# ay-lab/fithic

Measured on AMD Instinct MI355X. Metric: contact-pairs/sec through spline+p-value+BH pass (5 kb cis, whole node), higher is better.
Workload: dtype f64

## Files before the change

### fithic_amd/_capi.py

```python
import ctypes
import os
import subprocess

import numpy as np

from . import _loader

_PKG = os.path.dirname(os.path.abspath(__file__))
LIB_PATH = _loader.LIB_PATH
CSRC = os.path.join(_PKG, "csrc")

FHX_OK = 0
FHX_ERR_ARG, FHX_ERR_NO_DEVICE, FHX_ERR_HIP, FHX_ERR_UNSUPPORTED, FHX_ERR_REFERENCE_EXIT, FHX_ERR_NOMEM, FHX_ERR_INTERNAL = -1, -2, -3, -4, -5, -6, -7
MODE_INTRA_ONLY, MODE_INTER_ONLY, MODE_ALL = 0, 1, 2
TOTALS_REFERENCE, TOTALS_WIDE = 0, 1
INT64_MAX = (1 << 63) - 1

(A_HIST_SUMCC, A_HIST_NPAIRS, A_BIN_LB, A_BIN_UB, A_BIN_POSS, A_BIN_SUMCC, A_BIN_SUMDIST, A_BIN_POSS7, A_X, A_Y,
 A_KNOTS, A_COEFFS, A_TABLE_X, A_TABLE_Y0, A_TABLE_Y, A_OUTLIER_DIST_HIST, A_FDR_COUNTS, A_BIN_POSS0, A_DIST_KEYS,
 A_OUTLIER_DISTS) = range(20)
_ARRAY_DTYPE = {A_BIN_SUMDIST: np.float64, A_X: np.float64, A_Y: np.float64, A_KNOTS: np.float64,
                A_COEFFS: np.float64, A_TABLE_Y0: np.float64, A_TABLE_Y: np.float64}


# ... 73 lines not shown
    "fhx_reset_passes": (ctypes.c_int, [_P]),
    "fhx_get_stats": (ctypes.c_int, [_P, ctypes.POINTER(FhxStats)]),
    "fhx_fetch": (ctypes.c_int, [_P, _F64P, _F64P, _F64P, _F64P, _F64P]),
    "fhx_fetch_flags": (ctypes.c_int, [_P, ctypes.POINTER(ctypes.c_uint8), ctypes.POINTER(ctypes.c_uint8)]),
    "fhx_fetch_outlier_rows": (ctypes.c_int, [_P, ctypes.POINTER(ctypes.c_int64), ctypes.c_int64, ctypes.POINTER(ctypes.c_int64)]),
    "fhx_get_array": (ctypes.c_int, [_P, ctypes.c_int, _P, ctypes.c_int64, _I64P]),
    "fhx_device_ptr": (_P, [_P, ctypes.c_int]),
    "fhx_n_sorted": (ctypes.c_int64, [_P]),
    "fhx_bh_sort_stats": (ctypes.c_int, [_P, _I64P]),
    "fhx_k3_pass_info": (ctypes.c_int, [_P, _I64P]),
    "fhx_debug_k3_tiles_per_group": (ctypes.c_int, [_P, ctypes.c_int]),
    "fhx_debug_k1_wide": (ctypes.c_int, [_P, ctypes.c_int]),
    "fhx_k3_compact_variant": (ctypes.c_int, [_P, ctypes.POINTER(ctypes.c_int32)]),
    "fhx_kernel_seconds": (ctypes.c_int, [_P, _F64P, _F64P, _F64P]),
    "fhx_kernel_seconds_total": (ctypes.c_int, [_P, _F64P, _I64P, ctypes.c_int]),
    "fhx_kernel_events_dropped": (ctypes.c_int, [_P, _I64P]),
    "fhx_k2_heavy_launch": (ctypes.c_int, [_P, _F64P, _I64P]),
    "fhx_k2_heavy_clock": (ctypes.c_int, [_P, _F64P]),
    "fhx_k2_class_rows": (ctypes.c_int, [_P, _I64P]),
    "fhx_bdtrc_array": (ctypes.c_int, [_P, ctypes.c_double, _I32P, _F64P, ctypes.c_int64, _F64P]),
    "fhx_debug_format": (ctypes.c_int, [_P, _F64P, ctypes.c_int64, ctypes.c_int32, ctypes.c_char_p, _I32P]),
    "fhx_debug_contfrac": (ctypes.c_int, [_P, ctypes.c_int, ctypes.c_int, _F64P, _F64P, _F64P, ctypes.c_int64, _F64P]),
    "fhx_debug_lean_div": (ctypes.c_int, [_P, _F64P, _F64P, ctypes.c_int64, _F64P]),
    "fhx_debug_classify": (ctypes.c_int, [_P, ctypes.c_double, _I32P, _F64P, ctypes.c_int64, _I32P, _I32P, _F64P]),
    "fhx_debug_k2_rows": (ctypes.c_int, [_P, ctypes.c_double, ctypes.c_double, _I32P, _F64P, ctypes.POINTER(ctypes.c_uint8), ctypes.c_int64,
                                         ctypes.c_int32, _F64P, _I64P, _I64P, _I64P, ctypes.c_int64]),
    "fhx_bh_array": (ctypes.c_int, [_P, _F64P, ctypes.c_int64, ctypes.c_double, _F64P]),
    "fhx_bh_top_hist": (ctypes.c_int, [_P, _I64P, ctypes.c_int64]),
    "fhx_bh_set_cutoff": (ctypes.c_int, [_P, _I64P, ctypes.c_int64, ctypes.c_double]),
    "fhx_bh_top_hist_device": (ctypes.c_int, [_P]),
    "fhx_bh_set_cutoff_device": (ctypes.c_int, [_P, ctypes.c_double]),
    "fhx_bh_local_sort": (ctypes.c_int, [_P]),
    "fhx_bh_apply_sorted": (ctypes.c_int, [_P, _P, ctypes.c_int64, ctypes.c_int64, ctypes.c_double, ctypes.c_double, _P, _F64P]),
    "fhx_sort_u64": (ctypes.c_int, [_P, _P, ctypes.c_int64, _P, _P]),
    "fhx_bh_scatter": (ctypes.c_int, [_P, _P]),
    "fhx_memcpy_d2d": (ctypes.c_int, [_P, _P, _P, ctypes.c_int64]),
    "fhx_comm_unique_id": (ctypes.c_int, [_P, ctypes.c_int64]),
    "fhx_comm_init": (ctypes.c_int, [_P, _P, ctypes.c_int, ctypes.c_int]),
    "fhx_comm_init_custom": (ctypes.c_int, [_P, _P, ctypes.c_int, ctypes.c_int]),
    "fhx_comm_destroy": (ctypes.c_int, [_P]),
    "fhx_comm_info": (ctypes.c_int, [_P, ctypes.POINTER(ctypes.c_int), ctypes.POINTER(ctypes.c_int), ctypes.POINTER(ctypes.c_int)]),
    "fhx_run_pass_distributed": (ctypes.c_int, [_P, ctypes.POINTER(FhxFitInfo)]),
    "fhx_next_pass_distributed": (ctypes.c_int, [_P, _I64P]),
    "fhx_pass_stats_distributed": (ctypes.c_int, [_P, ctypes.POINTER(FhxStats)]),
    "fhx_bh_distributed": (ctypes.c_int, [_P, ctypes.c_double]),
    "fhx_dist_stage_seconds": (ctypes.c_int, [_P, _F64P]),
# ... 696 lines not shown
        return p, by_class, redo.value, hist

    def debug_contfrac(self, kind, lazy, a, b, x):
        a, b, x = (np.ascontiguousarray(v, np.float64) for v in (a, b, x))
        out = np.empty(len(a), np.float64)
        self._check(self._L.fhx_debug_contfrac(self._h, int(kind), int(lazy), _ptr(a, ctypes.c_double), _ptr(b, ctypes.c_double),
                                               _ptr(x, ctypes.c_double), len(a), _ptr(out, ctypes.c_double)))
        return out

    def debug_format(self, values, kind):
        v = np.ascontiguousarray(values, np.float64)
        text = ctypes.create_string_buffer(len(v) * 32)
        ln = np.empty(len(v), np.int32)
        self._check(self._L.fhx_debug_format(self._h, _ptr(v, ctypes.c_double), len(v), int(kind), text, _ptr(ln, ctypes.c_int32)))
        raw = text.raw
        return [raw[32 * i:32 * i + ln[i]] if ln[i] > 0 else None for i in range(len(v))]

    def debug_lean_div(self, n, d):
        n, d = (np.ascontiguousarray(v, np.float64) for v in (n, d))
        out = np.empty(len(n), np.float64)
        self._check(self._L.fhx_debug_lean_div(self._h, _ptr(n, ctypes.c_double), _ptr(d, ctypes.c_double), len(n), _ptr(out, ctypes.c_double)))
        return out

    def bh_array(self, p, n_total_tests):
        p = np.ascontiguousarray(p, np.float64)
        q = np.empty(len(p), np.float64)
        self._check(self._L.fhx_bh_array(self._h, _ptr(p, ctypes.c_double), len(p), float(n_total_tests), _ptr(q, ctypes.c_double)))
        return q

    def bh_top_hist(self):
        h = np.zeros(8192, np.int64)
        self._check(self._L.fhx_bh_top_hist(self._h, _ptr(h, ctypes.c_int64), len(h)))
        return h

    def bh_set_cutoff(self, global_hist, n_total_tests):
        h = np.ascontiguousarray(global_hist, np.int64)
        self._check(self._L.fhx_bh_set_cutoff(self._h, _ptr(h, ctypes.c_int64), len(h), float(n_total_tests)))

    def bh_top_hist_device(self):
        self._check(self._L.fhx_bh_top_hist_device(self._h))
        return self.device_ptr(4)

    def bh_set_cutoff_device(self, n_total_tests):
        self._check(self._L.fhx_bh_set_cutoff_device(self._h, float(n_total_tests)))

    def bh_local_sort(self):
# ... 668 lines not shown
```

### fithic_amd/csrc/fhx_bdtrc.hpp

```cpp
#pragma once
#include <hip/hip_runtime.h>
#include <cstdint>

namespace fhx {
namespace dev {

constexpr double kMachEp = 1.11022302462515654042E-16;
constexpr double kMaxLog = 7.09782712893383996732E2;
constexpr double kMinLog = -7.451332191019412076235E2;
constexpr double kMaxGam = 171.624376956302725;
constexpr double kBig = 4.503599627370496e15;
constexpr double kBigInv = 2.22044604925031308085e-16;

struct BinomTables {
    const double* lbeta;
    const double* inv_beta;
    double n;
    int small_n;
};

__device__ __forceinline__ double cephes_log1p(double x) {
    double z = 1.0 + x;
    if (z < 0.70710678118654752440 || z > 1.41421356237309504880) return log(z);
    z = x * x;
// ... 13 lines not shown
    z = -0.5 * z + x * (z * num / den);
    return x + z;
}

__device__ __forceinline__ double cephes_expm1(double x) {
    if (!isfinite(x)) {
        if (isnan(x) || x > 0) return x;
        return -1.0;
    }
    if (x < -0.5 || x > 0.5) return exp(x) - 1.0;
    const double xx = x * x;
    double ep = 1.2617719307481059087798E-4;
    ep = ep * xx + 3.0299440770744196129956E-2;
    ep = ep * xx + 9.9999999999999999991025E-1;
    double r = x * ep;
    double eq = 3.0019850513866445504159E-6;
    eq = eq * xx + 2.5244834034968410419224E-3;
    eq = eq * xx + 2.2726554820815502876593E-1;
    eq = eq * xx + 2.0000000000000000000897E0;
    r = r / (eq - r);
    return r + r;
}

template <bool SMALL_N = true>
__device__ __forceinline__ double pseries(double a, double b, double x, double lbeta_ab, double inv_beta_ab) {
    const double ai = 1.0 / a;
    double u = (1.0 - b) * x;
    double v = u / (a + 1.0);
    const double t1 = v;
    double t = u;
    double n = 2.0;
    double s = 0.0;
    const double z = kMachEp * ai;
    while (fabs(v) > z) {
        u = (n - b) * x / n;
        t *= u;
        v = t / (a + n);
        s += v;
        n += 1.0;
    }
    s += t1;
    s += ai;
    u = a * log(x);
    if (SMALL_N && (a + b) < kMaxGam && fabs(u) < kMaxLog) {
        t = inv_beta_ab;
        s = s * t * pow(x, a);
    } else {
        t = -lbeta_ab + u + log(s);
        s = (t < kMinLog) ? 0.0 : exp(t);
    }
    return s;
}

template <int KIND>
__device__ __forceinline__ double contfrac(double a, double b, double x) {
    double k1, k2, k3, k4, k5, k6, k7, k8, arg;
    if (KIND == 0) {
        arg = x;
        k1 = a; k2 = a + b; k3 = a; k4 = a + 1.0; k5 = 1.0; k6 = b - 1.0; k7 = k4; k8 = a + 2.0;
    } else {
        arg = x / (1.0 - x);
        k1 = a; k2 = b - 1.0; k3 = a; k4 = a + 1.0; k5 = 1.0; k6 = a + b; k7 = a + 1.0; k8 = a + 2.0;
    }
// ... 20 lines not shown
            t = 1.0;
        }
        if (t < thresh) break;

        k1 += 1.0;
        k2 += (KIND == 0) ? 1.0 : -1.0;
        k3 += 2.0;
        k4 += 2.0;
        k5 += 1.0;
        k6 += (KIND == 0) ? -1.0 : 1.0;
        k7 += 2.0;
        k8 += 2.0;

        if ((fabs(qk) + fabs(pk)) > kBig) {
            pkm2 *= kBigInv; pkm1 *= kBigInv; qkm2 *= kBigInv; qkm1 *= kBigInv;
        }
        if ((fabs(qk) < kBigInv) || (fabs(pk) < kBigInv)) {
            pkm2 *= kBig; pkm1 *= kBig; qkm2 *= kBig; qkm1 *= kBig;
        }
    } while (++n < 300);
    return ans;
}

__device__ __forceinline__ double lean_div(double n, double d) {
    const double y0 = __builtin_amdgcn_rcp(d);
    const double e0 = __builtin_fma(-d, y0, 1.0);
    const double y1 = __builtin_fma(y0, e0, y0);
    const double e1 = __builtin_fma(-d, y1, 1.0);
    const double y2 = __builtin_fma(y1, e1, y1);
    const double q0 = n * y2;
    const double r0 = __builtin_fma(-d, q0, n);
    return __builtin_fma(r0, y2, q0);
}

template <int MODE>
__device__ __forceinline__ double cf_div(double n, double d, double& y) {
    if (MODE == 0) return n / d;
    if (MODE == 1) return lean_div(n, d);
    double e = __builtin_fma(-d, y, 1.0);
    y = __builtin_fma(y, e, y);
    if (MODE == 2) {
        e = __builtin_fma(-d, y, 1.0);
        y = __builtin_fma(y, e, y);
    }
    const double q0 = n * y;
    const double r0 = __builtin_fma(-d, q0, n);
    return __builtin_fma(r0, y, q0);
}

template <int KIND, int MODE>
__device__ __forceinline__ double contfrac_lazy_impl(double a, double b, double arg) {
    double k1, k2, k3, k4, k5, k6, k8;
    if (KIND == 0) {
        k1 = a; k2 = a + b; k3 = a; k4 = a + 1.0; k5 = 1.0; k6 = b - 1.0; k8 = a + 2.0;
    } else {
        k1 = a; k2 = b - 1.0; k3 = a; k4 = a + 1.0; k5 = 1.0; k6 = a + b; k8 = a + 2.0;
    }
    double pkm2 = 0.0, qkm2 = 1.0, pkm1 = 1.0, qkm1 = 1.0;
    double rp = 1.0, rq = 1.0;
    double ans = 1.0, r = 1.0;
    bool fast_ok = true;
    const double thresh = 3.0 * kMachEp;
    double yrec = 0.0;
    if (MODE >= 2) {
        const double d0 = k3 * k4;
        yrec = __builtin_amdgcn_rcp(d0);
        double e0 = __builtin_fma(-d0, yrec, 1.0);
        yrec = __builtin_fma(yrec, e0, yrec);
        if (MODE == 3) {
            e0 = __builtin_fma(-d0, yrec, 1.0);
            yrec = __builtin_fma(yrec, e0, yrec);
        }
    }
    int n = 0;
    do {
        double xk = -cf_div<MODE>(arg * k1 * k2, k3 * k4, yrec);
        double pk = pkm1 + pkm2 * xk;
        double qk = qkm1 + qkm2 * xk;
        pkm2 = pkm1; pkm1 = pk; qkm2 = qkm1; qkm1 = qk;

        xk = cf_div<MODE>(arg * k5 * k6, k4 * k8, yrec);
        pk = pkm1 + pkm2 * xk;
        qk = qkm1 + qkm2 * xk;
        pkm2 = pkm1; pkm1 = pk; qkm2 = qkm1; qkm1 = qk;

        const double apk = fabs(pk), aqk = fabs(qk);
        const double mag_sum = aqk + apk;
        const double mag_min = fmin(apk, aqk);
        bool exact = true;
        if (__builtin_expect(fast_ok && mag_min > 1e-100 && mag_sum < 1e100, 1)) {
            const double c1 = rp * qk;
            const double c2 = pk * rq;
            if (__builtin_expect(fabs(c1 - c2) > 1e-13 * fabs(c2), 1)) {
                rp = pk;
                rq = qk;
                exact = false;
            }
        }
        if (__builtin_expect(exact, 0)) {
            if (fast_ok) {
                ans = rp / rq;
                r = ans;
            }
            double t;
            if (qk != 0) r = pk / qk;
            if (r != 0) {
                t = fabs((ans - r) / r);
                ans = r;
            } else {
                t = 1.0;
            }
            if (ans != r) fast_ok = false;
            rp = ans;
            rq = 1.0;
            if (t < thresh) break;
        }

        k1 += 1.0;
        k2 += (KIND == 0) ? 1.0 : -1.0;
        k3 += 2.0;
        k4 += 2.0;
        k5 += 1.0;
        k6 += (KIND == 0) ? -1.0 : 1.0;
        k8 += 2.0;

        if (__builtin_expect(mag_sum > kBig, 0)) {
            pkm2 *= kBigInv; pkm1 *= kBigInv; qkm2 *= kBigInv; qkm1 *= kBigInv;
        }
        if (__builtin_expect(mag_min < kBigInv, 0)) {
            pkm2 *= kBig; pkm1 *= kBig; qkm2 *= kBig; qkm1 *= kBig;
        }
    } while (++n < 300);
    return fast_ok ? rp / rq : ans;
}

template <int KIND>
__device__ __forceinline__ double contfrac_lazy(double a, double b, double x) {
    const double arg = (KIND == 0) ? x : x / (1.0 - x);
    const double aa = fabs(arg);
    if (aa > 1e-150 && aa < 1e150 && a >= 1.0 && a < 4.5e15 && b < 4.5e15) {
        if (a >= 2e8) return contfrac_lazy_impl<KIND, 3>(a, b, arg);
        if (a >= 1e6) return contfrac_lazy_impl<KIND, 2>(a, b, arg);
        return contfrac_lazy_impl<KIND, 1>(a, b, arg);
    }
    return contfrac_lazy_impl<KIND, 0>(a, b, arg);
}

struct CfRow {
    double k1, k2, k5, k6, d0, y0, d1, y1;
};
constexpr int kCfIters = 300;
constexpr double kCfLazyT = 1e-15;

typedef const CfRow __attribute__((address_space(4))) * CfRowConstPtr;

typedef double cf_d8 __attribute__((ext_vector_type(8)));
__device__ __forceinline__ CfRow cf_load_row(CfRowConstPtr p0) {
    const volatile cf_d8 __attribute__((address_space(4))) * p = (const volatile cf_d8 __attribute__((address_space(4))) *)p0;
    const cf_d8 v = *p;
    CfRow r;
    r.k1 = v[0]; r.k2 = v[1]; r.k5 = v[2]; r.k6 = v[3];
    r.d0 = v[4]; r.y0 = v[5]; r.d1 = v[6]; r.y1 = v[7];
    __builtin_amdgcn_sched_barrier(0);
    return r;
}

// ... 431 lines not shown
                                                double lbeta_ab, double inv_beta_ab) {
    double y = a * log(x);
    double t = b * log(xc);
    if (SMALL_N && (a + b) < kMaxGam && fabs(y) < kMaxLog && fabs(t) < kMaxLog) {
        t = pow(xc, b);
        t *= pow(x, a);
        t /= a;
        t *= w;
        t *= inv_beta_ab;
    } else {
        y += t - lbeta_ab;
        y += log(w / a);
        t = (y < kMinLog) ? 0.0 : exp(y);
    }
    if (flag == 1) {
        if (t <= kMachEp)
            t = 1.0 - kMachEp;
        else
            t = 1.0 - t;
    }
    return t;
}

template <int CLS, bool SMALL_N = true>
__device__ __forceinline__ double bdtrc_count_class(int count, const BinomTables& T, double p) {
    const double fk = (double)count - 1.0;
    const double aa = fk + 1.0, bb = T.n - fk, xx = p;
    const double lb = T.lbeta[count];
    const double ib = (SMALL_N && T.small_n) ? T.inv_beta[count] : 0.0;
    if (CLS == BC_PSERIES) {
        if (bb * xx <= 1.0 && xx <= 0.95) return pseries<SMALL_N>(aa, bb, xx, lb, ib);
        const double w = 1.0 - xx;
        double t = pseries<SMALL_N>(bb, aa, w, lb, ib);
        return (t <= kMachEp) ? 1.0 - kMachEp : 1.0 - t;
    }
    const double w1 = 1.0 - xx;
    if (CLS == BC_CF_BCF) return incbet_finish<SMALL_N>(aa, bb, xx, w1, contfrac_lazy<0>(aa, bb, xx), 0, lb, ib);
    if (CLS == BC_CF_SWAPPED) return incbet_finish<SMALL_N>(bb, aa, w1, xx, contfrac_lazy<0>(bb, aa, w1), 1, lb, ib);
    const int flag = (xx > aa / (aa + bb)) ? 1 : 0;
    const double a = flag ? bb : aa, b = flag ? aa : bb, x = flag ? w1 : xx, xc = flag ? xx : w1;
    return incbet_finish<SMALL_N>(a, b, x, xc, contfrac_lazy<1>(a, b, x) / xc, flag, lb, ib);
}

}
}
```

### fithic_amd/csrc/fhx_k2.hip

```cpp
#include "fhx_ctx.hpp"

namespace fhx {

__device__ __forceinline__ double prior_by_search(const K2Params& P, long long dist) {
    double look = (double)dist;
    if (look < P.min_x) look = P.min_x;
    if (look > P.max_x) look = P.max_x;
    int lo = 0, hi = P.n_table;
    while (lo < hi) {
        const int mid = (lo + hi) >> 1;
        if (P.table_x[mid] < look)
            lo = mid + 1;
        else
            hi = mid;
    }
    return P.table_y[min(lo, P.n_table - 1)];
}

template <int NF = -1>
__device__ __forceinline__ bool row_prior(const K2Params& P, int l1, int l2, double& prior, bool& is_inter) {
    const bool inter = l2 < 0;
    const int s2 = inter ? ~l2 : l2;
    const double b1 = P.no_bias ? 1.0 : P.slot_bias[l1], b2 = P.no_bias ? 1.0 : P.slot_bias[s2];
    if ((b1 < 0 || b2 < 0) && !inter) return false;
// ... 363 lines not shown
    }
    __device__ __forceinline__ Cursor open(unsigned int v) const {
        Cursor c;
        c.pr = pair_of(v);
        load(c);
        return c;
    }
    __device__ __forceinline__ const QEntry* at(const QSpan& q, Cursor& c, unsigned int v) const {
        if (v >= c.end) {
            do ++c.pr;
            while (v >= prefix[c.pr + 1]);
            load(c);
        }
        const unsigned int u = v - c.base;
        return u < c.c0 ? qentry(q, 2 * c.pr, (long long)u) : qentry(q, 2 * c.pr + 1, (long long)(u - c.c0));
    }
};
constexpr int K2_WAVES = K2_THREADS / 64;

template <int CLS, bool SMALL_N>
__global__ __launch_bounds__(K2_THREADS) void k2_queue(K2Params P, QSpan q) {
    __shared__ unsigned int hist_lds[K2_HIST_BINS];
    __shared__ unsigned int prefix_lds[QDense::PAIRS + 1], wave_tot[K2_WAVES];
    FusedHist H;
    H.init(hist_lds, P.top_hist);
    QDense D;
    D.build(q, prefix_lds, wave_tot);
    const unsigned long long total = D.total();
    const unsigned int lane = threadIdx.x & 63;
    const unsigned long long n_waves = (unsigned long long)gridDim.x * K2_WAVES;
    const unsigned long long share = ((total + n_waves - 1) / n_waves + 63ull) & ~63ull;
    const unsigned long long begin = ((unsigned long long)blockIdx.x * K2_WAVES + (threadIdx.x >> 6)) * share;
    const unsigned long long end = min(total, begin + share);
    QDense::Cursor cur{0, 0u, 0u, 0u};
    if (begin + lane < end) cur = D.open((unsigned int)(begin + lane));
#pragma unroll 1
    for (unsigned long long v = begin + lane; v < end; v += 64) {
        const QEntry e = *D.at(q, cur, (unsigned int)v);
        const bool is_inter = e.count < 0;
        const int c = is_inter ? -e.count : e.count;
        const double pv = dev::bdtrc_count_class<CLS, SMALL_N>(c, is_inter ? P.inter : P.intra, e.prior);
        store_p<false>(P.p + e.row, pv);
        H.add(pv);
    }
    H.flush(P.top_hist);
}

constexpr int K2_SORT_TILE = 1024;
constexpr int K2_SORT_BUCKETS = 32;
template <int CLS, bool SMALL_N, int WPE>
__global__ __launch_bounds__(K2_THREADS) __attribute__((amdgpu_waves_per_eu(WPE))) void k2_queue_by_count(K2Params P, QSpan q,
                                                                                                         unsigned int* next_tile) {
    static_assert(K2_SORT_TILE == 4 * K2_THREADS, "four entries per thread");
    __shared__ QEntry tile[K2_SORT_TILE];
    __shared__ unsigned int bucket_cnt[K2_SORT_BUCKETS], bucket_off[K2_SORT_BUCKETS];
    __shared__ unsigned int hist_lds[K2_HIST_BINS];
    __shared__ unsigned int prefix_lds[QDense::PAIRS + 1], wave_tot[K2_WAVES], tile_lds;
    FusedHist H;
    H.init(hist_lds, P.top_hist);
    QDense D;
    D.build(q, prefix_lds, wave_tot);
    const unsigned int total = D.total();
    const unsigned int share = (total + gridDim.x - 1) / gridDim.x;
    const unsigned int rounds = max(1u, (share + K2_SORT_TILE - 1) / K2_SORT_TILE);
    const unsigned int tile_n = max(min((unsigned int)K2_SORT_TILE, ((share + rounds - 1) / rounds + 63u) & ~63u), 64u);
    const unsigned int tiles = (total + tile_n - 1) / tile_n;
    unsigned int mine = blockIdx.x;
    for (;;) {
        if (threadIdx.x < K2_SORT_BUCKETS) bucket_cnt[threadIdx.x] = 0;
        if (threadIdx.x == 0) tile_lds = mine;
        __syncthreads();
        const unsigned int t = tile_lds;
        if (t >= tiles) break;
        if (threadIdx.x == 0) mine = gridDim.x + atomicAdd(next_tile, 1u);
        const unsigned int v0 = t * tile_n;
        const int m = (int)min(tile_n, total - v0);
        QEntry e[4];
        int bucket[4];
        unsigned int slot[4];
        QDense::Cursor cur{0, 0u, 0u, 0u};
// ... 7 lines not shown
                const int c = e[r].count < 0 ? -e[r].count : e[r].count;
                bucket[r] = c < K2_SORT_BUCKETS - 1 ? c : K2_SORT_BUCKETS - 1;
                slot[r] = atomicAdd(&bucket_cnt[bucket[r]], 1u);
            }
        }
        __syncthreads();
        if (threadIdx.x < K2_SORT_BUCKETS) {
            unsigned int off = 0;
            for (int b = 0; b < (int)threadIdx.x; ++b) off += bucket_cnt[b];
            bucket_off[threadIdx.x] = off;
        }
        __syncthreads();
#pragma unroll
        for (int r = 0; r < 4; ++r)
            if (bucket[r] >= 0) tile[bucket_off[bucket[r]] + slot[r]] = e[r];
        __syncthreads();
#pragma unroll 1
        for (int r = 0; r < 4; ++r) {
            const int idx = r * K2_THREADS + threadIdx.x;
            if (idx < m) {
                const QEntry x = tile[idx];
                const bool is_inter = x.count < 0;
                const int c = is_inter ? -x.count : x.count;
                const double pv = dev::bdtrc_count_class<CLS, SMALL_N>(c, is_inter ? P.inter : P.intra, x.prior);
                store_p<false>(P.p + x.row, pv);
                H.add(pv);
            }
        }
        __syncthreads();
    }
    H.flush(P.top_hist);
}



__device__ __forceinline__ int k2h_bucket(int signed_count) {
    const bool inter = signed_count < 0;
    const int c = inter ? -signed_count : signed_count;
    return c < K2H_KCAP ? (inter ? K2H_KCAP + c : c) : K2H_GENERIC;
}

__global__ __launch_bounds__(K2H_THREADS) void k2h_scatter(QSpan q, const unsigned int* __restrict__ block_hist,
                                                           const unsigned int* __restrict__ off, QEntry* __restrict__ out) {
    __shared__ unsigned int cursor[K2H_BUCKETS];
    for (int d = threadIdx.x; d < K2H_BUCKETS; d += K2H_THREADS) cursor[d] = off[d] + block_hist[(size_t)d * K2H_BLOCKS + blockIdx.x];
    __syncthreads();
    for (int sh = blockIdx.x; sh < q.n_shards; sh += K2H_BLOCKS) {
// ... 180 lines not shown
    unsigned long long at = tile_offsets[blockIdx.x] + fhxscan::block_exclusive_scan(c, &total);
    for (int k = 0; k < fhxscan::SCAN_ITEMS; ++k)
        if (base + k < n && flag[base + k]) rows[at++] = base + k;
}

__global__ void k_bdtrc_array(dev::BinomTables T, const int32_t* __restrict__ count, const double* __restrict__ prior,
                              int64_t n, double* __restrict__ out) {
    const int64_t stride = (int64_t)gridDim.x * blockDim.x;
    for (int64_t i = (int64_t)blockIdx.x * blockDim.x + threadIdx.x; i < n; i += stride)
        out[i] = dev::bdtrc_count(count[i], T, prior[i]);
}

template <int KIND, int LAZY>
__global__ void k_debug_contfrac(const double* __restrict__ a, const double* __restrict__ b, const double* __restrict__ x,
                                 int64_t n, double* __restrict__ out) {
    const int64_t stride = (int64_t)gridDim.x * blockDim.x;
    for (int64_t i = (int64_t)blockIdx.x * blockDim.x + threadIdx.x; i < n; i += stride)
        out[i] = LAZY ? dev::contfrac_lazy<KIND>(a[i], b[i], x[i]) : dev::contfrac<KIND>(a[i], b[i], x[i]);
}

__global__ void k_debug_lean_div(const double* __restrict__ n, const double* __restrict__ d, int64_t len, double* __restrict__ out) {
    const int64_t stride = (int64_t)gridDim.x * blockDim.x;
    for (int64_t i = (int64_t)blockIdx.x * blockDim.x + threadIdx.x; i < len; i += stride) out[i] = dev::lean_div(n[i], d[i]);
}

__global__ __launch_bounds__(256) void k2_memo_rows(int n_d, int lo_idx, int cap, int with_inter, int32_t* __restrict__ loc1,
                                                   int32_t* __restrict__ loc2, int32_t* __restrict__ count, int64_t n_v) {
    const int64_t stride = (int64_t)gridDim.x * blockDim.x;
    const int64_t intra = (int64_t)n_d * (cap + 1);
    for (int64_t i = (int64_t)blockIdx.x * blockDim.x + threadIdx.x; i < n_v; i += stride) {
        if (i < intra) {
            const int d = lo_idx + (int)(i / (cap + 1));
            loc1[i] = 0;
            loc2[i] = d;
            count[i] = (int)(i % (cap + 1));
        } else {
            loc1[i] = 0;
            loc2[i] = ~0;
            count[i] = (int)(i - intra);
        }
        (void)with_inter;
    }
}

__global__ __launch_bounds__(256) void k2_memo_gather(K2Params P, const double* __restrict__ table, int n_d, int cap, int has_intra,
                                                     int has_inter, unsigned int* __restrict__ overflow_rows,
// ... 227 lines not shown
    static_assert((K2H_BLOCKS & (K2H_BLOCKS - 1)) == 0, "shard -> column by masking");
    Q->heavy_hist = plan.legacy_heavy ? nullptr : ctx->d_block_hist;
    if (Q->heavy_hist && !prezeroed)
        FHX_HIP(hipMemsetAsync(ctx->d_block_hist, 0, (size_t)K2H_BUCKETS * K2H_BLOCKS * sizeof(unsigned int), ctx->stream));
    ctx->k2_shards = plan.n_shards;
    auto span = [&](int cls, QEntry* buf, int dir) {
        Q->q[cls - 1] = QSpan{dir > 0 ? buf : buf + plan.cap_s - 1, plan.cap_s, dir, plan.n_shards, Q->count + (size_t)(cls - 1) * K2_MAX_SHARDS};
    };
    span(dev::BC_CF_SWAPPED, ctx->d_queue[0], 1);
    span(dev::BC_PSERIES, ctx->d_queue[0], -1);
    span(dev::BC_CF_BCF, ctx->d_queue[1], 1);
    span(dev::BC_CF_BD, ctx->d_queue[1], -1);
    span(K2_CLOSED, ctx->d_queue_sorted, 1);
    return FHX_OK;
}

template <int CLS, bool SMALL_N>
static void launch_k2_queue(fhx_ctx* ctx, const K2Params& P, const K2Queues& Q) {
    hipLaunchKernelGGL(HIP_KERNEL_NAME(k2_queue<CLS, SMALL_N>), dim3(2 * resident_grid(ctx, k2_queue<CLS, SMALL_N>)), dim3(K2_THREADS), 0,
                       ctx->stream, P, Q.q[CLS - 1]);
}
template <int CLS, bool SMALL_N>
static void launch_k2_queue_by_count(fhx_ctx* ctx, const K2Params& P, const K2Queues& Q) {
    constexpr int PIECE = SMALL_N ? 4 : 5;
    hipLaunchKernelGGL(HIP_KERNEL_NAME(k2_queue_by_count<CLS, SMALL_N, PIECE>), dim3(resident_grid(ctx, k2_queue_by_count<CLS, SMALL_N, PIECE>)),
                       dim3(K2_THREADS), 0, ctx->stream, P, Q.q[CLS - 1], (unsigned int*)(ctx->d_words->k2_next + CLS));
}
template <int ROWS, int WAVES, bool SMALL_N>
static void launch_k2h_heavy(fhx_ctx* ctx, const K2Params& P, QEntry* redo) {
    hipLaunchKernelGGL(HIP_KERNEL_NAME(k2h_heavy<ROWS, WAVES, SMALL_N>), dim3(256 * WAVES), dim3(K2H_THREADS), 0, ctx->stream,
                       K2HeavyParams{P.intra, P.inter, P.p, P.top_hist}, (const QEntry*)ctx->d_queue_sorted, (const unsigned int*)ctx->d_k2h_off,
                       (const unsigned int*)ctx->d_digit_total, (const dev::CfRow*)ctx->d_cf_tab, redo, &ctx->d_words->k2_redo,
                       (unsigned int*)ctx->d_words->k2_next);
}

template <bool SMALL_N>
static int launch_k2(fhx_ctx* ctx, const K2Plan& plan, const K2Params& P, const K2Queues& Q) {
    const dim3 cgrid(plan.n_shards), block(K2_THREADS);
    if (P.nonfixed)
        hipLaunchKernelGGL(HIP_KERNEL_NAME(k2_classify<1, 4, 0>), cgrid, block, 0, ctx->stream, P, Q);
    else
        hipLaunchKernelGGL(HIP_KERNEL_NAME(k2_classify<0, 4, 3, true, true>), cgrid, block, 0, ctx->stream, P, Q);
    hipLaunchKernelGGL(k2_closed, dim3(256 * 8), block, 0, ctx->stream, P, Q.q[K2_CLOSED - 1], &ctx->d_words->k2_redo, &ctx->d_words->bh_cutoff);
    if (plan.legacy_heavy) {
        FHX_HIP(hipEventRecord(ctx->ev[6], ctx->stream));
        launch_k2_queue<dev::BC_CF_SWAPPED, SMALL_N>(ctx, P, Q);
        FHX_HIP(hipEventRecord(ctx->ev[7], ctx->stream));
// ... 298 lines not shown
    if (thr5) FHX_HIP(hipMemcpyAsync(thr5, d_thr, (size_t)n * 40, hipMemcpyDeviceToHost, ctx->stream));
    FHX_HIP(hipStreamSynchronize(ctx->stream));
    return FHX_OK;
}

int fhx_debug_lean_div(fhx_ctx* ctx, const double* n, const double* d, int64_t len, double* out) {
    if (!ctx || !n || !d || !out || len < 0) return FHX_ERR_ARG;
    if (ctx->device < 0) return fail(ctx, FHX_ERR_NO_DEVICE, "host-only context");
    if (len == 0) return FHX_OK;
    FHX_HIP(hipSetDevice(ctx->device));
    double* dv[3] = {nullptr, nullptr, nullptr};
    const size_t bytes = (size_t)len * sizeof(double);
    for (int k = 0; k < 3; ++k) FHX_HIP(hipMalloc(&dv[k], bytes));
    FHX_HIP(hipMemcpyAsync(dv[0], n, bytes, hipMemcpyHostToDevice, ctx->stream));
    FHX_HIP(hipMemcpyAsync(dv[1], d, bytes, hipMemcpyHostToDevice, ctx->stream));
    hipLaunchKernelGGL(k_debug_lean_div, dim3(grid_for(len, 256)), dim3(256), 0, ctx->stream, dv[0], dv[1], len, dv[2]);
    FHX_HIP(hipGetLastError());
    FHX_HIP(hipMemcpyAsync(out, dv[2], bytes, hipMemcpyDeviceToHost, ctx->stream));
    FHX_HIP(hipStreamSynchronize(ctx->stream));
    for (int k = 0; k < 3; ++k) dev_free(dv[k]);
    return FHX_OK;
}

int fhx_next_pass(fhx_ctx* ctx, int64_t* n_outliers_total) {
    if (!ctx) return FHX_ERR_ARG;
    if (ctx->device < 0) return fail(ctx, FHX_ERR_NO_DEVICE, "host-only context");
    if (!ctx->have_p) return fail(ctx, FHX_ERR_ARG, "fhx_pvalues must run first");
    FHX_HIP(hipSetDevice(ctx->device));
    unsigned long long* n_out = &ctx->d_words->outliers_added;
    unsigned long long* first_dup = &ctx->d_words->first_dup;
    FHX_HIP(hipMemsetAsync(n_out, 0, sizeof(unsigned long long), ctx->stream));
    FHX_HIP(hipMemsetAsync(first_dup, 0xFF, sizeof(unsigned long long), ctx->stream));
    if (ctx->nonfixed) {
        hipLaunchKernelGGL(nf_fold_outliers, dim3(grid_for(ctx->n_rows, 256)), dim3(256), 0, ctx->stream, ctx->d_loc1, ctx->d_loc2,
                           ctx->d_p, 1.0 / ctx->fit.bh_total_tests, ctx->d_skip, ctx->n_rows,
                           (const int32_t*)ctx->d_slot_mid, ctx->d_keys[0], n_out, first_dup, (const long long*)ctx->d_grow);
        FHX_HIP(hipGetLastError());
        unsigned long long added = 0, dup = ~0ull;
        FHX_HIP(hipMemcpyAsync(&added, n_out, sizeof(added), hipMemcpyDeviceToHost, ctx->stream));
        FHX_HIP(hipMemcpyAsync(&dup, first_dup, sizeof(dup), hipMemcpyDeviceToHost, ctx->stream));
        FHX_HIP(hipStreamSynchronize(ctx->stream));
        std::vector<int64_t> fresh((size_t)added);
        if (added) {
            FHX_HIP(hipMemcpyAsync(fresh.data(), ctx->d_keys[0], (size_t)added * sizeof(int64_t), hipMemcpyDeviceToHost, ctx->stream));
            FHX_HIP(hipStreamSynchronize(ctx->stream));
        }
// ... 164 lines not shown
```

### include/fithic_mi355x.h

```cpp
#ifndef FITHIC_MI355X_H
#define FITHIC_MI355X_H

#include <stdint.h>

#ifdef __cplusplus
extern "C" {
#endif

#define FHX_OK 0
#define FHX_ERR_ARG (-1)
#define FHX_ERR_NO_DEVICE (-2)
#define FHX_ERR_HIP (-3)
#define FHX_ERR_UNSUPPORTED (-4)
#define FHX_ERR_REFERENCE_EXIT (-5)
#define FHX_ERR_NOMEM (-6)
#define FHX_ERR_INTERNAL (-7)

#define FHX_MODE_INTRA_ONLY 0
#define FHX_MODE_INTER_ONLY 1
#define FHX_MODE_ALL 2

#define FHX_TOTALS_REFERENCE 0
#define FHX_TOTALS_WIDE 1

// ... 149 lines not shown
int fhx_debug_k3_tiles_per_group(fhx_ctx* ctx, int per);
int fhx_debug_k1_wide(fhx_ctx* ctx, int on);
int fhx_kernel_seconds(fhx_ctx* ctx, double* k1, double* k2, double* k3);
int fhx_kernel_seconds_total(fhx_ctx* ctx, double* sums4, int64_t* counts4, int reset);
int fhx_kernel_events_dropped(fhx_ctx* ctx, int64_t* dropped4);
int fhx_k2_heavy_launch(fhx_ctx* ctx, double* seconds, int64_t* rows);
int fhx_k2_heavy_clock(fhx_ctx* ctx, double* ghz);
int fhx_k2_class_rows(fhx_ctx* ctx, int64_t* out5);

int fhx_bh_array(fhx_ctx* ctx, const double* p, int64_t n, double n_total_tests, double* q);

int fhx_bdtrc_array(fhx_ctx* ctx, double n_total, const int32_t* count, const double* prior, int64_t n, double* out);

int fhx_debug_k2_rows(fhx_ctx* ctx, double n_intra, double n_inter, const int32_t* count, const double* prior, const uint8_t* is_inter,
                      int64_t n, int32_t nonfixed, double* p_out, int64_t* class_rows5, int64_t* n_redo, int64_t* top_hist,
                      int64_t hist_cap);

int fhx_debug_contfrac(fhx_ctx* ctx, int kind, int lazy, const double* a, const double* b, const double* x, int64_t n,
                       double* out);

int fhx_debug_classify(fhx_ctx* ctx, double n_total, const int32_t* count, const double* prior, int64_t n, int32_t* by_table,
                       int32_t* by_arith, double* thr5);
int fhx_debug_lean_div(fhx_ctx* ctx, const double* n, const double* d, int64_t len, double* out);
int fhx_debug_format(fhx_ctx* ctx, const double* values, int64_t n, int32_t kind, char* text32, int32_t* len);

int fhx_bh_top_hist(fhx_ctx* ctx, int64_t* hist_out, int64_t capacity);
int fhx_bh_set_cutoff(fhx_ctx* ctx, const int64_t* global_hist, int64_t n_bins, double n_total_tests);
int fhx_bh_top_hist_device(fhx_ctx* ctx);
int fhx_bh_set_cutoff_device(fhx_ctx* ctx, double n_total_tests);
int fhx_bh_local_sort(fhx_ctx* ctx);
int fhx_bh_apply_sorted(fhx_ctx* ctx, const void* d_sorted_keys, int64_t n, int64_t global_rank0,
                        double carry_in, double n_total_tests, void* d_q_sorted, double* block_max_out);
int fhx_sort_u64(fhx_ctx* ctx, const void* d_keys_in, int64_t n, void* d_keys_out, void* d_perm_out);
int fhx_bh_scatter(fhx_ctx* ctx, const void* d_q_sorted_local);
int fhx_memcpy_d2d(fhx_ctx* ctx, void* dst, const void* src, int64_t bytes);

#define FHX_UNIQUE_ID_BYTES 128
int fhx_comm_unique_id(void* id_out, int64_t capacity);
int fhx_comm_init(fhx_ctx* ctx, const void* rccl_unique_id, int rank, int nranks);
typedef struct fhx_transport {
    void* user;
    int (*all_reduce_i64)(void* user, void* d_buf, int64_t n, int op);
    int (*all_gather)(void* user, const void* d_send, void* d_recv, int64_t bytes);
    int (*all_to_all_v)(void* user, const void* d_send, const int64_t* send_counts, const int64_t* send_offsets, void* d_recv,
                        const int64_t* recv_counts, const int64_t* recv_offsets, int elem_bytes);
} fhx_transport;
// ... 240 lines not shown
```

Before: 13.95 billion.

## Replace f64 divisions in pseries and continued fraction with LDS reciprocal tables

Builds per-block shared-memory tables of reciprocals, 1/j for the power series and 1/(j(j+1)) for the continued fraction. Integer-indexed denominators in the incomplete beta loops then use a table lookup plus one Newton-corrected quotient instead of a full f64 divide. The continued fraction uses lean_div on a narrower magnitude window and falls back to exact division when it leaves that window. It also adds a debug entry point to check the table quotients, and changes the piece size for the CF_BD queue kernel. The aim is to cut expensive double-precision division latency in the p-value kernels, at the cost of extra LDS, table build work at each kernel start, and possible last-bit numeric differences.

```diff
diff --git a/fithic_amd/_capi.py b/fithic_amd/_capi.py
--- a/fithic_amd/_capi.py
+++ b/fithic_amd/_capi.py
@@ -119,6 +119,7 @@
     "fhx_debug_format": (ctypes.c_int, [_P, _F64P, ctypes.c_int64, ctypes.c_int32, ctypes.c_char_p, _I32P]),
     "fhx_debug_contfrac": (ctypes.c_int, [_P, ctypes.c_int, ctypes.c_int, _F64P, _F64P, _F64P, ctypes.c_int64, _F64P]),
     "fhx_debug_lean_div": (ctypes.c_int, [_P, _F64P, _F64P, ctypes.c_int64, _F64P]),
+    "fhx_debug_table_div": (ctypes.c_int, [_P, ctypes.c_int, _F64P, ctypes.c_int64, _F64P, _I32P]),
     "fhx_debug_classify": (ctypes.c_int, [_P, ctypes.c_double, _I32P, _F64P, ctypes.c_int64, _I32P, _I32P, _F64P]),
     "fhx_debug_k2_rows": (ctypes.c_int, [_P, ctypes.c_double, ctypes.c_double, _I32P, _F64P, ctypes.POINTER(ctypes.c_uint8), ctypes.c_int64,
                                          ctypes.c_int32, _F64P, _I64P, _I64P, _I64P, ctypes.c_int64]),
@@ -861,6 +862,17 @@
         self._check(self._L.fhx_debug_lean_div(self._h, _ptr(n, ctypes.c_double), _ptr(d, ctypes.c_double), len(n), _ptr(out, ctypes.c_double)))
         return out
 
+    def debug_table_div(self, kind, num):
+        num = np.ascontiguousarray(num, np.float64)
+        length = ctypes.c_int32(0)
+        dummy = np.empty(1, np.float64)
+        self._check(self._L.fhx_debug_table_div(self._h, int(kind), _ptr(dummy, ctypes.c_double), 0, _ptr(dummy, ctypes.c_double), ctypes.byref(length)))
+        out = np.empty((length.value - 1, len(num)), np.float64)
+        if len(num):
+            self._check(self._L.fhx_debug_table_div(self._h, int(kind), _ptr(num, ctypes.c_double), len(num), _ptr(out, ctypes.c_double),
+                                                    ctypes.byref(length)))
+        return out
+
     def bh_array(self, p, n_total_tests):
         p = np.ascontiguousarray(p, np.float64)
         q = np.empty(len(p), np.float64)
diff --git a/fithic_amd/csrc/fhx_bdtrc.hpp b/fithic_amd/csrc/fhx_bdtrc.hpp
--- a/fithic_amd/csrc/fhx_bdtrc.hpp
+++ b/fithic_amd/csrc/fhx_bdtrc.hpp
@@ -59,23 +59,53 @@
     return r + r;
 }
 
-template <bool SMALL_N = true>
-__device__ __forceinline__ double pseries(double a, double b, double x, double lbeta_ab, double inv_beta_ab) {
-    const double ai = 1.0 / a;
-    double u = (1.0 - b) * x;
-    double v = u / (a + 1.0);
-    const double t1 = v;
-    double t = u;
-    double n = 2.0;
-    double s = 0.0;
-    const double z = kMachEp * ai;
-    while (fabs(v) > z) {
-        u = (n - b) * x / n;
-        t *= u;
-        v = t / (a + n);
-        s += v;
-        n += 1.0;
-    }
+__device__ __forceinline__ double lean_rcp(double d);
+__device__ __forceinline__ double lean_quot(double n, double d, double y);
+constexpr int kPsTabJ = 512;
+template <bool SMALL_N = true, bool LEAN = false>
+__device__ __forceinline__ double pseries(double a, double b, double x, double lbeta_ab, double inv_beta_ab, const double* rtab = nullptr) {
+    double ai, t1, s = 0.0;
+    if (LEAN && x > 1e-150 && x <= 0.95 && b * x <= 1.0 && a >= 1.0 && a < 4.5e15 && b >= 1.0 && b < 4.5e15 && b == __builtin_rint(b)) {
+        int ja = kPsTabJ;
+        if (a < (double)kPsTabJ) {
+            const int ia = (int)a;
+            if ((double)ia == a) ja = ia;
+        }
+        const double a1 = a + 1.0;
+        ai = lean_quot(1.0, a, ja < kPsTabJ ? rtab[ja] : lean_rcp(a));
+        double u = (1.0 - b) * x;
+        double v = lean_quot(u, a1, ja + 1 < kPsTabJ ? rtab[ja + 1] : lean_rcp(a1));
+        t1 = v;
+        double t = u;
+        double n = 2.0;
+        int ni = 2;
+        const double z = kMachEp * ai;
+        while (fabs(v) > z) {
+            u = lean_quot((n - b) * x, n, ni < kPsTabJ ? rtab[ni] : lean_rcp(n));
+            t *= u;
+            const double an = a + n;
+            v = lean_quot(t, an, ja + ni < kPsTabJ ? rtab[ja + ni] : lean_rcp(an));
+            s += v;
+            n += 1.0;
+            ni += 1;
+        }
+    } else {
+        ai = 1.0 / a;
+        double u = (1.0 - b) * x;
+        double v = u / (a + 1.0);
+        t1 = v;
+        double t = u;
+        double n = 2.0;
+        const double z = kMachEp * ai;
+        while (fabs(v) > z) {
+            u = (n - b) * x / n;
+            t *= u;
+            v = t / (a + n);
+            s += v;
+            n += 1.0;
+        }
+    }
+    double u, t;
     s += t1;
     s += ai;
     u = a * log(x);
@@ -142,15 +172,32 @@
     return ans;
 }
 
-__device__ __forceinline__ double lean_div(double n, double d) {
+__device__ __forceinline__ double lean_rcp(double d) {
     const double y0 = __builtin_amdgcn_rcp(d);
     const double e0 = __builtin_fma(-d, y0, 1.0);
     const double y1 = __builtin_fma(y0, e0, y0);
     const double e1 = __builtin_fma(-d, y1, 1.0);
-    const double y2 = __builtin_fma(y1, e1, y1);
+    return __builtin_fma(y1, e1, y1);
+}
+__device__ __forceinline__ double lean_div(double n, double d) {
+    const double y2 = lean_rcp(d);
     const double q0 = n * y2;
     const double r0 = __builtin_fma(-d, q0, n);
     return __builtin_fma(r0, y2, q0);
+}
+__device__ __forceinline__ double lean_quot(double n, double d, double y) {
+    const double q0 = n * y;
+    const double r0 = __builtin_fma(d, q0, -n);
+    return __builtin_fma(-r0, y, q0);
+}
+
+constexpr int kCfTabJ = 448;
+template <bool PRODUCT>
+__device__ __forceinline__ void div_table_build(double* tab, int len) {
+    for (int j = (int)threadIdx.x; j < len; j += (int)blockDim.x) {
+        const double fj = (double)j;
+        tab[j] = j == 0 ? 0.0 : lean_rcp(PRODUCT ? fj * (fj + 1.0) : fj);
+    }
 }
 
 template <int MODE>
@@ -168,8 +215,12 @@
     return __builtin_fma(r0, y, q0);
 }
 
-template <int KIND, int MODE>
-__device__ __forceinline__ double contfrac_lazy_impl(double a, double b, double arg) {
+template <int KIND, int MODE, bool LEAN = false>
+__device__ __forceinline__ double contfrac_lazy_impl(double a, double b, double arg, const double* ytab = nullptr) {
+    static_assert(!LEAN || MODE >= 1, "MODE 0 is the loop for operands outside lean_div's window");
+    constexpr bool TAB = LEAN && MODE == 1;
+    constexpr double kWinLo = LEAN ? 1e-30 : 1e-100, kWinHi = LEAN ? 1e30 : 1e100;
+    bool lean_live = true;
     double k1, k2, k3, k4, k5, k6, k8;
     if (KIND == 0) {
         k1 = a; k2 = a + b; k3 = a; k4 = a + 1.0; k5 = 1.0; k6 = b - 1.0; k8 = a + 2.0;
@@ -192,14 +243,40 @@
             yrec = __builtin_fma(yrec, e0, yrec);
         }
     }
+    int tj = kCfTabJ;
+    double ty0 = 0.0, ty1 = 0.0;
+    if (TAB) {
+        if (a < (double)(kCfTabJ - 1)) {
+            const int ia = (int)a;
+            if ((double)ia == a) tj = ia;
+        }
+        const int jc = tj < kCfTabJ - 2 ? tj : kCfTabJ - 2;
+        ty0 = ytab[jc];
+        ty1 = ytab[jc + 1];
+    }
     int n = 0;
     do {
-        double xk = -cf_div<MODE>(arg * k1 * k2, k3 * k4, yrec);
+        double y0 = ty0, y1 = ty1;
+        double xk;
+        if (TAB) {
+            const double d0 = k3 * k4;
+            if (__builtin_expect(tj > kCfTabJ - 2, 0)) {
+                y0 = lean_rcp(d0);
+                y1 = lean_rcp(k4 * k8);
+            }
+            tj += 2;
+            const int jc = tj < kCfTabJ - 2 ? tj : kCfTabJ - 2;
+            ty0 = ytab[jc];
+            ty1 = ytab[jc + 1];
+            xk = -lean_quot(arg * k1 * k2, d0, y0);
+        } else {
+            xk = -cf_div<MODE>(arg * k1 * k2, k3 * k4, yrec);
+        }
         double pk = pkm1 + pkm2 * xk;
         double qk = qkm1 + qkm2 * xk;
         pkm2 = pkm1; pkm1 = pk; qkm2 = qkm1; qkm1 = qk;
 
-        xk = cf_div<MODE>(arg * k5 * k6, k4 * k8, yrec);
+        xk = TAB ? lean_quot(arg * k5 * k6, k4 * k8, y1) : cf_div<MODE>(arg * k5 * k6, k4 * k8, yrec);
         pk = pkm1 + pkm2 * xk;
         qk = qkm1 + qkm2 * xk;
         pkm2 = pkm1; pkm1 = pk; qkm2 = qkm1; qkm1 = qk;
@@ -208,7 +285,8 @@
         const double mag_sum = aqk + apk;
         const double mag_min = fmin(apk, aqk);
         bool exact = true;
-        if (__builtin_expect(fast_ok && mag_min > 1e-100 && mag_sum < 1e100, 1)) {
+        const bool win = fast_ok && mag_min > kWinLo && mag_sum < kWinHi;
+        if (__builtin_expect(win, 1)) {
             const double c1 = rp * qk;
             const double c2 = pk * rq;
             if (__builtin_expect(fabs(c1 - c2) > 1e-13 * fabs(c2), 1)) {
@@ -218,19 +296,28 @@
             }
         }
         if (__builtin_expect(exact, 0)) {
-            if (fast_ok) {
-                ans = rp / rq;
-                r = ans;
-            }
             double t;
-            if (qk != 0) r = pk / qk;
-            if (r != 0) {
-                t = fabs((ans - r) / r);
+            if (LEAN && win && lean_live) {
+                ans = rp;
+                if (rq != 1.0) ans = lean_div(rp, rq);
+                r = lean_div(pk, qk);
+                t = fabs(lean_div(ans - r, r));
                 ans = r;
             } else {
-                t = 1.0;
+                lean_live = false;
+                if (fast_ok) {
+                    ans = rp / rq;
+                    r = ans;
+                }
+                if (qk != 0) r = pk / qk;
+                if (r != 0) {
+                    t = fabs((ans - r) / r);
+                    ans = r;
+                } else {
+                    t = 1.0;
+                }
+                if (ans != r) fast_ok = false;
             }
-            if (ans != r) fast_ok = false;
             rp = ans;
             rq = 1.0;
             if (t < thresh) break;
@@ -251,17 +338,21 @@
             pkm2 *= kBig; pkm1 *= kBig; qkm2 *= kBig; qkm1 *= kBig;
         }
     } while (++n < 300);
+    if (LEAN && fast_ok) {
+        if (rq == 1.0) return rp;
+        if (lean_live) return lean_div(rp, rq);
+    }
     return fast_ok ? rp / rq : ans;
 }
 
-template <int KIND>
-__device__ __forceinline__ double contfrac_lazy(double a, double b, double x) {
+template <int KIND, bool LEAN = false>
+__device__ __forceinline__ double contfrac_lazy(double a, double b, double x, const double* ytab = nullptr) {
     const double arg = (KIND == 0) ? x : x / (1.0 - x);
     const double aa = fabs(arg);
     if (aa > 1e-150 && aa < 1e150 && a >= 1.0 && a < 4.5e15 && b < 4.5e15) {
-        if (a >= 2e8) return contfrac_lazy_impl<KIND, 3>(a, b, arg);
-        if (a >= 1e6) return contfrac_lazy_impl<KIND, 2>(a, b, arg);
-        return contfrac_lazy_impl<KIND, 1>(a, b, arg);
+        if (a >= 2e8) return contfrac_lazy_impl<KIND, 3, LEAN>(a, b, arg);
+        if (a >= 1e6) return contfrac_lazy_impl<KIND, 2, LEAN>(a, b, arg);
+        return contfrac_lazy_impl<KIND, 1, LEAN>(a, b, arg, ytab);
     }
     return contfrac_lazy_impl<KIND, 0>(a, b, arg);
 }
@@ -739,25 +830,33 @@
     return t;
 }
 
-template <int CLS, bool SMALL_N = true>
-__device__ __forceinline__ double bdtrc_count_class(int count, const BinomTables& T, double p) {
+template <int CLS, bool SMALL_N = true, bool LEAN = false>
+__device__ __forceinline__ double bdtrc_count_class(int count, const BinomTables& T, double p, const double* tab = nullptr) {
+    static_assert(!LEAN || CLS == BC_PSERIES || CLS == BC_CF_BCF || CLS == BC_CF_BD, "the swapped class has no small divisors");
     const double fk = (double)count - 1.0;
     const double aa = fk + 1.0, bb = T.n - fk, xx = p;
     const double lb = T.lbeta[count];
     const double ib = (SMALL_N && T.small_n) ? T.inv_beta[count] : 0.0;
     if (CLS == BC_PSERIES) {
-        if (bb * xx <= 1.0 && xx <= 0.95) return pseries<SMALL_N>(aa, bb, xx, lb, ib);
+        if (LEAN) {
+            const bool direct = bb * xx <= 1.0 && xx <= 0.95;
+            const double w = 1.0 - xx;
+            const double t = pseries<SMALL_N, true>(direct ? aa : bb, direct ? bb : aa, direct ? xx : w, lb, ib, tab);
+            if (direct) return t;
+            return (t <= kMachEp) ? 1.0 - kMachEp : 1.0 - t;
+        }
+        if (bb * xx <= 1.0 && xx <= 0.95) return pseries<SMALL_N, LEAN>(aa, bb, xx, lb, ib, tab);
         const double w = 1.0 - xx;
-        double t = pseries<SMALL_N>(bb, aa, w, lb, ib);
+        double t = pseries<SMALL_N, LEAN>(bb, aa, w, lb, ib, tab);
         return (t <= kMachEp) ? 1.0 - kMachEp : 1.0 - t;
     }
     const double w1 = 1.0 - xx;
-    if (CLS == BC_CF_BCF) return incbet_finish<SMALL_N>(aa, bb, xx, w1, contfrac_lazy<0>(aa, bb, xx), 0, lb, ib);
+    if (CLS == BC_CF_BCF) return incbet_finish<SMALL_N>(aa, bb, xx, w1, contfrac_lazy<0, LEAN>(aa, bb, xx, tab), 0, lb, ib);
     if (CLS == BC_CF_SWAPPED) return incbet_finish<SMALL_N>(bb, aa, w1, xx, contfrac_lazy<0>(bb, aa, w1), 1, lb, ib);
     const int flag = (xx > aa / (aa + bb)) ? 1 : 0;
     const double a = flag ? bb : aa, b = flag ? aa : bb, x = flag ? w1 : xx, xc = flag ? xx : w1;
-    return incbet_finish<SMALL_N>(a, b, x, xc, contfrac_lazy<1>(a, b, x) / xc, flag, lb, ib);
-}
-
-}
-}
+    return incbet_finish<SMALL_N>(a, b, x, xc, contfrac_lazy<1, LEAN>(a, b, x, tab) / xc, flag, lb, ib);
+}
+
+}
+}
diff --git a/fithic_amd/csrc/fhx_k2.hip b/fithic_amd/csrc/fhx_k2.hip
--- a/fithic_amd/csrc/fhx_k2.hip
+++ b/fithic_amd/csrc/fhx_k2.hip
@@ -409,6 +409,9 @@
 __global__ __launch_bounds__(K2_THREADS) void k2_queue(K2Params P, QSpan q) {
     __shared__ unsigned int hist_lds[K2_HIST_BINS];
     __shared__ unsigned int prefix_lds[QDense::PAIRS + 1], wave_tot[K2_WAVES];
+    constexpr bool LEAN = CLS == dev::BC_PSERIES;
+    __shared__ double rtab[LEAN ? dev::kPsTabJ : 1];
+    if (LEAN) dev::div_table_build<false>(rtab, dev::kPsTabJ);
     FusedHist H;
     H.init(hist_lds, P.top_hist);
     QDense D;
@@ -426,7 +429,7 @@
         const QEntry e = *D.at(q, cur, (unsigned int)v);
         const bool is_inter = e.count < 0;
         const int c = is_inter ? -e.count : e.count;
-        const double pv = dev::bdtrc_count_class<CLS, SMALL_N>(c, is_inter ? P.inter : P.intra, e.prior);
+        const double pv = dev::bdtrc_count_class<CLS, SMALL_N, LEAN>(c, is_inter ? P.inter : P.intra, e.prior, rtab);
         store_p<false>(P.p + e.row, pv);
         H.add(pv);
     }
@@ -443,6 +446,8 @@
     __shared__ unsigned int bucket_cnt[K2_SORT_BUCKETS], bucket_off[K2_SORT_BUCKETS];
     __shared__ unsigned int hist_lds[K2_HIST_BINS];
     __shared__ unsigned int prefix_lds[QDense::PAIRS + 1], wave_tot[K2_WAVES], tile_lds;
+    __shared__ double ytab[dev::kCfTabJ];
+    dev::div_table_build<true>(ytab, dev::kCfTabJ);
     FusedHist H;
     H.init(hist_lds, P.top_hist);
     QDense D;
@@ -496,7 +501,7 @@
                 const QEntry x = tile[idx];
                 const bool is_inter = x.count < 0;
                 const int c = is_inter ? -x.count : x.count;
-                const double pv = dev::bdtrc_count_class<CLS, SMALL_N>(c, is_inter ? P.inter : P.intra, x.prior);
+                const double pv = dev::bdtrc_count_class<CLS, SMALL_N, true>(c, is_inter ? P.inter : P.intra, x.prior, ytab);
                 store_p<false>(P.p + x.row, pv);
                 H.add(pv);
             }
@@ -723,6 +728,18 @@
 __global__ void k_debug_lean_div(const double* __restrict__ n, const double* __restrict__ d, int64_t len, double* __restrict__ out) {
     const int64_t stride = (int64_t)gridDim.x * blockDim.x;
     for (int64_t i = (int64_t)blockIdx.x * blockDim.x + threadIdx.x; i < len; i += stride) out[i] = dev::lean_div(n[i], d[i]);
+}
+
+template <bool PRODUCT, int LEN>
+__global__ __launch_bounds__(256) void k_debug_table_div(const double* __restrict__ num, int64_t m, double* __restrict__ out) {
+    __shared__ double tab[LEN];
+    dev::div_table_build<PRODUCT>(tab, LEN);
+    __syncthreads();
+    const int j = (int)blockIdx.x + 1;
+    if (j >= LEN) return;
+    const double fj = (double)j;
+    const double d = PRODUCT ? fj * (fj + 1.0) : fj;
+    for (int64_t i = threadIdx.x; i < m; i += blockDim.x) out[(int64_t)(j - 1) * m + i] = dev::lean_quot(num[i], d, tab[j]);
 }
 
 __global__ __launch_bounds__(256) void k2_memo_rows(int n_d, int lo_idx, int cap, int with_inter, int32_t* __restrict__ loc1,
@@ -996,7 +1013,7 @@
 }
 template <int CLS, bool SMALL_N>
 static void launch_k2_queue_by_count(fhx_ctx* ctx, const K2Params& P, const K2Queues& Q) {
-    constexpr int PIECE = SMALL_N ? 4 : 5;
+    constexpr int PIECE = (SMALL_N || CLS == dev::BC_CF_BD) ? 4 : 5;
     hipLaunchKernelGGL(HIP_KERNEL_NAME(k2_queue_by_count<CLS, SMALL_N, PIECE>), dim3(resident_grid(ctx, k2_queue_by_count<CLS, SMALL_N, PIECE>)),
                        dim3(K2_THREADS), 0, ctx->stream, P, Q.q[CLS - 1], (unsigned int*)(ctx->d_words->k2_next + CLS));
 }
@@ -1341,6 +1358,30 @@
     return FHX_OK;
 }
 
+int fhx_debug_table_div(fhx_ctx* ctx, int kind, const double* num, int64_t m, double* out, int32_t* table_len) {
+    if (!ctx || (kind != 0 && kind != 1) || !num || !out || !table_len || m < 0) return FHX_ERR_ARG;
+    if (ctx->device < 0) return fail(ctx, FHX_ERR_NO_DEVICE, "host-only context");
+    const int len = kind == 0 ? dev::kCfTabJ : dev::kPsTabJ;
+    *table_len = len;
+    if (m == 0) return FHX_OK;
+    FHX_HIP(hipSetDevice(ctx->device));
+    double *d_num = nullptr, *d_out = nullptr;
+    const size_t out_bytes = (size_t)(len - 1) * (size_t)m * sizeof(double);
+    FHX_HIP(hipMalloc(&d_num, (size_t)m * sizeof(double)));
+    FHX_HIP(hipMalloc(&d_out, out_bytes));
+    FHX_HIP(hipMemcpyAsync(d_num, num, (size_t)m * sizeof(double), hipMemcpyHostToDevice, ctx->stream));
+    if (kind == 0)
+        hipLaunchKernelGGL(HIP_KERNEL_NAME(k_debug_table_div<true, dev::kCfTabJ>), dim3(len - 1), dim3(256), 0, ctx->stream, d_num, m, d_out);
+    else
+        hipLaunchKernelGGL(HIP_KERNEL_NAME(k_debug_table_div<false, dev::kPsTabJ>), dim3(len - 1), dim3(256), 0, ctx->stream, d_num, m, d_out);
+    FHX_HIP(hipGetLastError());
+    FHX_HIP(hipMemcpyAsync(out, d_out, out_bytes, hipMemcpyDeviceToHost, ctx->stream));
+    FHX_HIP(hipStreamSynchronize(ctx->stream));
+    dev_free(d_num);
+    dev_free(d_out);
+    return FHX_OK;
+}
+
 int fhx_next_pass(fhx_ctx* ctx, int64_t* n_outliers_total) {
     if (!ctx) return FHX_ERR_ARG;
     if (ctx->device < 0) return fail(ctx, FHX_ERR_NO_DEVICE, "host-only context");
diff --git a/include/fithic_mi355x.h b/include/fithic_mi355x.h
--- a/include/fithic_mi355x.h
+++ b/include/fithic_mi355x.h
@@ -195,6 +195,7 @@
 int fhx_debug_classify(fhx_ctx* ctx, double n_total, const int32_t* count, const double* prior, int64_t n, int32_t* by_table,
                        int32_t* by_arith, double* thr5);
 int fhx_debug_lean_div(fhx_ctx* ctx, const double* n, const double* d, int64_t len, double* out);
+int fhx_debug_table_div(fhx_ctx* ctx, int kind, const double* num, int64_t m, double* out, int32_t* table_len);
 int fhx_debug_format(fhx_ctx* ctx, const double* values, int64_t n, int32_t kind, char* text32, int32_t* len);
 
 int fhx_bh_top_hist(fhx_ctx* ctx, int64_t* hist_out, int64_t capacity);
```

Measured after the change: 14.09 billion, median of 6. +1.0%, better.
